# ceres-solver/ceres-solver

Measured on NVIDIA H100. Metric: lm_iterations_per_sec, higher is better.
Workload: dtype f64

## Files before the change

### ceres_solver_b200/csrc/b200ba.cu

```cuda
#include <algorithm>
#include <array>
#include <cmath>
#include <cstdarg>
#include <cstdio>
#include <cstdlib>
#include <cstring>
#include <limits>
#include <numeric>
#include <string>
#include <vector>

#ifdef B200_WITH_NCCL
#include <dlfcn.h>
#include <nccl.h>
#endif

#include "../../include/b200ba.h"
#include "kernels.cuh"
#include "kernels_v2.cuh"
#include "kernels_v2b.cuh"
#include "kernels_v4b.cuh"
#include "pmv_kernels.cuh"
#include "vector_kernels.cuh"
#include "cg_kernel.cuh"
// ... 189 lines not shown
  void* cusolver = nullptr;
  int num_huge = 0;
  int* d_huge_pts = nullptr;
  bool residuals_resident = false;
  double *d_ftf_inv = nullptr, *d_spse[3] = {nullptr, nullptr, nullptr};
  double *d_pq_parts = nullptr, *d_seed_pq = nullptr;
  int num_cam_items = 0;
  CamItem* d_cam_items = nullptr;
  int* d_cam_rows = nullptr;
  double* d_q3 = nullptr;
  bool xs = false;
  bool xs_ready = false;
  bool xs_diag_ready = false;
  int xs_grid = 0;
  XsView xsv{};
  int num_xs_long = 0, num_xs_short = 0;
  int* d_xs_order = nullptr;
  bool xs_pcg = false;
  XsPcgArgs xpa{};
  size_t xs_pcg_smem = 0;
  std::vector<int> h_cam_idx, h_pt_idx, h_pt_ptr;
  bool sp_ready = false;
  bool xs_arrays = false;
  SparseView spv{};
  long long sp_storage = 0;
  int sp_grid = 0;
  size_t sp_smem = 0;
  int* d_sp_cnt_init = nullptr;
  double* d_red = nullptr;
  bool xchg_ok = false;
  uint4* d_xchg = nullptr;
  XchgPeers xpeers{};
// ... 254 lines not shown
  OK(launch(h, K_SQNORM, [&] {
    sqnorm_kernel<<<h->grid_tile[K_SQNORM], kTile, tile_smem_bytes<3, 1>(), h->stream>>>(h->view, d_out);
  }));
  return allreduce_sum(h, d_out + 3 * static_cast<size_t>(h->P), 9 * static_cast<size_t>(h->C));
}

int scale_dev(b200_handle* h, const double* d_scale) {
  h->xs_ready = false;
  return launch(h, K_SCALE, [&] {
    scale_kernel<<<flat_grid(h, 12 * static_cast<size_t>(h->N), 256), 256, 0, h->stream>>>(h->view, d_scale);
  });
}

int xs_assemble_dev(b200_handle* h) {
  OK(launch(h, K_DIAG_BLOCKS, [&] {
    if (h->num_xs_long > 0)
      xs_assemble_kernel<true><<<std::min(h->num_xs_long, h->sm_count * 32), kXsAsmThreads, 0, h->stream>>>(
          h->xsv, h->view, h->d_xs_order, h->num_xs_long, h->d_ete_inv, h->d_upper45);
    if (h->num_xs_short > 0)
      xs_assemble_kernel<false><<<std::min((h->num_xs_short + kXsAsmThreads / 32 - 1) / (kXsAsmThreads / 32), h->sm_count * 32),
                                  kXsAsmThreads, 0, h->stream>>>(h->xsv, h->view, h->d_xs_order + h->num_xs_long, h->num_xs_short,
                                                                 h->d_ete_inv, h->d_upper45);
  }));
  h->xs_ready = true;
  h->xs_diag_ready = true;
  return B200_OK;
}

int schur_init_dev(b200_handle* h, const double* d_b, const double* d_D) {
  SchurState st{};
  st.b = d_b;
  st.D = d_D;
  st.ete_inv = h->d_ete_inv;
  st.rhs = h->d_rhs;
  st.ye = h->d_ye;
  CU(cudaMemsetAsync(h->d_rhs, 0, sizeof(double) * 9 * h->C, h->stream));
  h->q_from_init = false;
// ... 386 lines not shown
  summary->num_iterations = 1;
  summary->residual_norm = 0.0;
  if (h->h_fail[0] != 0 || h->h_fail[1] != 0) {
    summary->termination_type = B200_LS_FAILURE;
    return B200_OK;
  }
  summary->termination_type = B200_LS_SUCCESS;
  OK(back_substitute_dev(h, d_b, h->d_sol, d_x));
  CU(cudaMemcpyAsync(d_x + 3 * static_cast<size_t>(h->P), h->d_sol, sizeof(double) * n, cudaMemcpyDeviceToDevice, h->stream));
  return B200_OK;
}

constexpr double kFactorMaxBytes = 48.0 * (1ull << 30);
static_assert(kSpMaxCols == 9 * kSnMaxCams && kSpThreads == 32 * 8 && kSpTileRows == 64,
              "an update tile: two column blocks per warp, two rows per lane");
int sparse_analyse(b200_handle* h) {
  XsPattern xp;
  xs_pattern(h->C, h->N, h->h_cam_idx.data(), h->h_pt_idx.data(), h->h_pt_ptr.data(), &xp);
  SparsePlan sp;
  plan_sparse_schur(h->C, xp.blk_row, xp.blk_col, &sp);
  if (8.0 * static_cast<double>(sp.storage) > kFactorMaxBytes)
    return fail(B200_ERR_UNSUPPORTED, "sparse factor of %d cameras needs %.1f GB", h->C, 8.0 * static_cast<double>(sp.storage) / 1e9);
  if (!h->xs_arrays) {
    XsView& x = h->xsv;
    x.C = h->C;
    x.num_blocks = static_cast<int>(xp.blk_row.size());
    OK(upload(h, xp.blk_row, &x.blk_row));
    OK(upload(h, xp.blk_col, &x.blk_col));
    OK(upload(h, xp.pair_ptr, &x.pair_ptr));
    OK(upload(h, xp.pairs, &x.pairs));
    OK(dev_alloc(h, &x.S, 81 * static_cast<size_t>(x.num_blocks)));
    std::vector<int> order;
    h->num_xs_long = xs_assembly_order(xp, &order);
    h->num_xs_short = x.num_blocks - h->num_xs_long;
    OK(upload(h, order, &h->d_xs_order));
    h->xs_arrays = true;
  }
  SparseView& v = h->spv;
  v.C = h->C;
  v.ns = sp.ns;
  OK(upload(h, sp.pinv, &v.pinv));
  OK(upload(h, sp.sn_first, &v.sn_first));
  OK(upload(h, sp.row_ptr, &v.row_ptr));
  OK(upload(h, sp.rows, &v.rows));
  OK(upload(h, sp.val, &v.val));
  OK(upload(h, sp.upd_ptr, &v.upd_ptr));
  OK(upload(h, sp.upd, &v.upd));
  OK(upload(h, sp.ntf_ptr, &v.ntf_ptr));
  OK(upload(h, sp.ntf, &v.ntf));
  OK(upload(h, sp.blk_off, &v.blk_off));
// ... 322 lines not shown
  OK(raise_smem_limit(cam_blocks_v2_kernel<true>, (kCamBlkThreads / 32) * kCamBlkWarpBytes));
  OK(raise_smem_limit(cam_blocks_v2_kernel<false>, (kCamBlkThreads / 32) * kCamBlkWarpBytes));
  OK(raise_smem_limit(jtj_v2_kernel, lim));
  OK(raise_smem_limit(schur_mul_v3_kernel, lim));
  OK(raise_smem_limit(schur_init_v4_kernel<true>, lim));
  OK(raise_smem_limit(schur_init_v4_kernel<false>, lim));
  OK(raise_smem_limit(jtj_v4_kernel<true>, lim));
  OK(raise_smem_limit(jtj_v4_kernel<false>, lim));
  OK(raise_smem_limit(schur_mul_v4_kernel<true>, lim));
  OK(raise_smem_limit(schur_mul_v4_kernel<false>, lim));
  OK(raise_smem_limit(evaluate_v2_kernel<true>, lim));
  OK(raise_smem_limit(evaluate_v2_kernel<false>, lim));
  OK(raise_smem_limit(diag_blocks_v2_kernel<true>, lim));
  OK(raise_smem_limit(diag_blocks_v2_kernel<false>, lim));
  OK(raise_smem_limit(xs_pcg_kernel, lim));
  OK(raise_smem_limit(sparse_factor_kernel, lim));
  return B200_OK;
}

struct StepResult {
  b200_solver_summary ls{};
  double model_cost_change = 0.0;
  double step_sq = 0.0, x_sq = 0.0;
  bool finite = true;
};

struct DeviceSide {
  b200_handle* h;
  const b200_lm_options* opt;
  int np, vgrid;
// ... 742 lines not shown
      OK(upload(h, std::vector<int2>(pl.num_ctas, make_int2(0, 0)), &h->v2_mul.cta_big));
    }
    h->v2_smem = pl.v2_smem;
    h->mul_smem = pl.mul_smem;
    h->eval_v2_smem = pl.eval_smem;
    h->diag_v2_smem = pl.diag_smem;
    h->diag_v2_replicas = pl.diag_replicas;
  }
  if (h->xs) {
    const XsPattern& xp = pl.xp;
    XsView& x = h->xsv;
    x.C = C;
    x.num_blocks = static_cast<int>(xp.blk_row.size());
    OK(upload(h, xp.blk_row, &x.blk_row));
    OK(upload(h, xp.blk_col, &x.blk_col));
    OK(upload(h, xp.pair_ptr, &x.pair_ptr));
    OK(upload(h, xp.pairs, &x.pairs));
    OK(upload(h, xp.cols, &x.cols));
    OK(upload(h, xp.col_ptr, &x.col_ptr));
    OK(upload(h, pl.xs_steps, &x.steps));
    OK(upload(h, pl.xs_warp_step, &x.warp_step));
    OK(dev_alloc(h, &x.S, 81 * static_cast<size_t>(x.num_blocks)));
    OK(dev_alloc(h, &x.T, 9 * static_cast<size_t>(xp.off_blocks)));
    OK(upload(h, pl.xs_order, &h->d_xs_order));
    h->num_xs_long = pl.num_xs_long;
    h->num_xs_short = x.num_blocks - pl.num_xs_long;
    h->xs_grid = pl.xs_grid;
    h->xs_pcg = pl.xs_pcg;
    if (h->xs_pcg) {
      XsPcgArgs& a = h->xpa;
      a.v = x;
      OK(upload(h, pl.xs_pcg_cta, &a.cta));
      OK(upload(h, pl.xs_pcg_warp_step, &a.warp_step));
      OK(upload(h, pl.xs_pcg_fptr, &a.fptr));
      OK(upload(h, pl.xs_pcg_fcol, &a.fcol));
      OK(upload(h, pl.xs_pcg_cols, &a.v.cols));
      a.max_blocks = pl.xs_pcg_max_blocks;
      a.max_cams = pl.xs_pcg_max_cams;
      a.max_foreign = pl.xs_pcg_max_foreign;
      a.max_steps = pl.xs_pcg_max_cta_steps;
      a.stage_slots = pl.xs_pcg_stage_slots;
// ... 492 lines not shown
```

### ceres_solver_b200/csrc/common.cuh

```cuda
#pragma once
#include <cuda_runtime.h>
#include <stdint.h>

namespace b200 {

constexpr int kTile = 128;

struct TileDesc {
  int obs_begin = 0;
  int obs_count = 0;
  int pt_begin = 0;
  int pt_count = 0;
  int chunk = 0;
};

struct ProblemView {
  int C, P;
  int N;
  int num_tiles;
  const TileDesc* tiles;
  const int* cam_idx;
  const int* pt_ptr;
  const int* pt_of_row;
  const double* obs;
  double* values;
  __device__ __host__ double* E() const { return values; }
  __device__ __host__ double* F() const { return values + 6 * static_cast<size_t>(N); }
};

__device__ __forceinline__ uint32_t smem_u32(const void* p) {
  return static_cast<uint32_t>(__cvta_generic_to_shared(p));
}
__device__ __forceinline__ void mbar_init(uint64_t* bar, uint32_t count) {
  asm volatile("mbarrier.init.shared::cta.b64 [%0], %1;" ::"r"(smem_u32(bar)), "r"(count));
}
__device__ __forceinline__ void fence_mbar_init() {
  asm volatile("fence.mbarrier_init.release.cluster;" ::: "memory");
}
__device__ __forceinline__ void mbar_arrive_expect_tx(uint64_t* bar, uint32_t bytes) {
  asm volatile("mbarrier.arrive.expect_tx.shared::cta.b64 _, [%0], %1;" ::"r"(smem_u32(bar)), "r"(bytes)
               : "memory");
}
__device__ __forceinline__ bool mbar_try_wait(uint64_t* bar, uint32_t parity) {
  uint32_t ok;
  asm volatile(
      "{\n"
      ".reg .pred p;\n"
// ... 136 lines not shown
```

### ceres_solver_b200/csrc/explicit_schur.cuh

```cuda
#pragma once
#include "common.cuh"

namespace b200 {

constexpr int kXsThreads = 256;
constexpr int kXsWarps = kXsThreads / 32;
constexpr int kXsMinCtas = 2;
constexpr int kXsStep = 3;
constexpr int kXsAsmThreads = 256;
constexpr int kXsLongPairs = 96;
constexpr int kXsStepCountShift = 27;
constexpr int kXsStepFirst = 1 << 29;
constexpr int kXsStepLast = 1 << 30;

struct XsView {
  int C;
  int num_blocks;
  const int* blk_row;
  const int* blk_col;
  const int* pair_ptr;
  const int2* pairs;
  const int2* cols;
  const int* col_ptr;
  const int2* steps;
  const int* warp_step;
  double* S;
  double* T;
};

__device__ __forceinline__ void xs_pairs(const XsView& v, const ProblemView& p, const double* __restrict__ ete_inv, int q_begin,
                                         int q_end, int lane, double& acc0, double& acc1, double& acc2) {
  const double* __restrict__ E = p.E();
  const double* __restrict__ F = p.F();
  const bool owner = lane < 27;
  const int u = owner ? lane / 3 : 0, w0 = owner ? 3 * (lane - 3 * (lane / 3)) : 0;
  const int q = lane >> 2, ga = (lane >> 1) & 1, gc = lane & 1;
  for (int q0 = q_begin; q0 < q_end; q0 += 8) {
    const int nq = min(8, q_end - q0);
    int r = 0, s = 0;
    double g = 0.0;
    if (q < nq) {
      const int2 rs = __ldg(v.pairs + q0 + q);
      r = rs.x;
      s = rs.y;
      const double* er = E + 6 * static_cast<size_t>(r) + 3 * ga;
      const double* es = E + 6 * static_cast<size_t>(s) + 3 * gc;
      const double e0 = es[0], e1 = es[1], e2 = es[2], f0 = er[0], f1 = er[1], f2 = er[2];
      const double* pp = ete_inv + 6 * static_cast<size_t>(__ldg(p.pt_of_row + r));
      const double P00 = pp[0], P01 = pp[1], P02 = pp[2], P11 = pp[3], P12 = pp[4], P22 = pp[5];
      const double pe0 = P00 * e0 + P01 * e1 + P02 * e2;
      const double pe1 = P01 * e0 + P11 * e1 + P12 * e2;
      const double pe2 = P02 * e0 + P12 * e1 + P22 * e2;
      g = f0 * pe0 + f1 * pe1 + f2 * pe2;
      if (r == s && ga == gc) g -= 1.0;
    }
    for (int t0 = 0; t0 < nq; t0 += 4) {
      double fr[4][2], fs[4][6], gg[4][4];
#pragma unroll
      for (int t = 0; t < 4; ++t) {
        const int src = 4 * (t0 + t);
#pragma unroll
        for (int k = 0; k < 4; ++k) gg[t][k] = __shfl_sync(0xffffffffu, g, (src + k) & 31);
        const int rr = __shfl_sync(0xffffffffu, r, src & 31), ss = __shfl_sync(0xffffffffu, s, src & 31);
        const double* pr = F + 18 * static_cast<size_t>(rr) + u;
        const double* ps = F + 18 * static_cast<size_t>(ss) + w0;
        fr[t][0] = pr[0];
        fr[t][1] = pr[9];
#pragma unroll
        for (int m = 0; m < 3; ++m) {
          fs[t][m] = ps[m];
          fs[t][3 + m] = ps[9 + m];
        }
      }
#pragma unroll
      for (int t = 0; t < 4; ++t) {
        if (t0 + t >= nq) continue;
        const double a0 = gg[t][0] * fr[t][0] + gg[t][2] * fr[t][1], a1 = gg[t][1] * fr[t][0] + gg[t][3] * fr[t][1];
#pragma unroll
        acc0 -= a0 * fs[t][0] + a1 * fs[t][3];
        acc1 -= a0 * fs[t][1] + a1 * fs[t][4];
        acc2 -= a0 * fs[t][2] + a1 * fs[t][5];
      }
    }
  }
}

template <bool kLong>
__global__ void __launch_bounds__(kXsAsmThreads) xs_assemble_kernel(XsView v, ProblemView p, const int* __restrict__ blocks,
                                                                   int num, const double* __restrict__ ete_inv,
                                                                   double* __restrict__ upper45) {
  __shared__ double s_part[kLong ? kXsAsmThreads / 32 : 1][81];
  const int lane = threadIdx.x & 31, warp = threadIdx.x >> 5;
  const bool owner = lane < 27;
  const int u = owner ? lane / 3 : 0, w0 = owner ? 3 * (lane - 3 * (lane / 3)) : 0;
  const int item0 = kLong ? static_cast<int>(blockIdx.x) : static_cast<int>(blockIdx.x) * (kXsAsmThreads / 32) + warp;
  const int items = kLong ? static_cast<int>(gridDim.x) : static_cast<int>(gridDim.x) * (kXsAsmThreads / 32);
  for (int it = item0; it < num; it += items) {
    const int b = __ldg(blocks + it);
    const int p0 = __ldg(v.pair_ptr + b), p1 = __ldg(v.pair_ptr + b + 1);
    double acc[3] = {0.0, 0.0, 0.0};
    if (kLong) {
      constexpr int W = kXsAsmThreads / 32;
      const int n = p1 - p0;
      xs_pairs(v, p, ete_inv, p0 + static_cast<int>(static_cast<long long>(n) * warp / W),
               p0 + static_cast<int>(static_cast<long long>(n) * (warp + 1) / W), lane, acc[0], acc[1], acc[2]);
      __syncthreads();
      if (owner)
#pragma unroll
        for (int m = 0; m < 3; ++m) s_part[warp][9 * u + w0 + m] = acc[m];
      __syncthreads();
      if (warp != 0) continue;
      if (owner)
#pragma unroll
        for (int m = 0; m < 3; ++m) {
          double t = 0.0;
#pragma unroll
          for (int k = 0; k < W; ++k) t += s_part[k][9 * u + w0 + m];
          acc[m] = t;
        }
    } else {
      xs_pairs(v, p, ete_inv, p0, p1, lane, acc[0], acc[1], acc[2]);
    }
    if (owner) {
      double* sb = v.S + 81 * static_cast<size_t>(b) + 9 * u + w0;
      sb[0] = acc[0];
      sb[1] = acc[1];
      sb[2] = acc[2];
      const int i = __ldg(v.blk_row + b);
      if (upper45 != nullptr && __ldg(v.blk_col + b) == i) {
        double* o = upper45 + 45 * static_cast<size_t>(i) + u * 9 - u * (u - 1) / 2 - u;
        if (u <= w0) o[w0] = acc[0];
        if (u <= w0 + 1) o[w0 + 1] = acc[1];
        if (u <= w0 + 2) o[w0 + 2] = acc[2];
      }
    }
  }
}

struct XsStepData {
  int2 d;
  int2 c;
  double s[9];
};
template <bool kShared>
__device__ __forceinline__ int2 xs_step_desc(const XsView& v, int k, int k1) {
  return k < k1 ? (kShared ? v.steps[k] : __ldg(v.steps + k)) : make_int2(0, 0);
}
__device__ __forceinline__ bool xs_lane_in(int2 d, int e) { return e < ((d.y >> kXsStepCountShift) & 3); }
template <bool kShared>
__device__ __forceinline__ int2 xs_step_col(const XsView& v, int2 d, int e) {
// ... 147 lines not shown
```

### ceres_solver_b200/csrc/kernels_v4b.cuh

```cuda
#pragma once
#include "kernels_v2b.cuh"

namespace b200 {

__device__ __forceinline__ void invert_sym3_llt_rsqrt(const double m[6], double inv[6]) {
  const double i00 = rsqrt(m[0]);
  const double l10 = m[1] * i00, l20 = m[2] * i00;
  const double i11 = rsqrt(m[3] - l10 * l10);
  const double l21 = (m[4] - l20 * l10) * i11;
  const double i22 = rsqrt(m[5] - l20 * l20 - l21 * l21);
  const double i10 = -l10 * i00 * i11;
  const double i21 = -l21 * i11 * i22;
  const double i20 = -(l20 * i00 + l21 * i10) * i22;
  inv[0] = i00 * i00 + i10 * i10 + i20 * i20;
  inv[1] = i10 * i11 + i20 * i21;
  inv[2] = i20 * i22;
  inv[3] = i11 * i11 + i21 * i21;
  inv[4] = i21 * i22;
  inv[5] = i22 * i22;
}

struct InitV4Args {
  const double* b;
  const double* D;
// ... 280 lines not shown
    if (static_cast<int>(threadIdx.x) >= d.obs_count) continue;
    const size_t r = static_cast<size_t>(d.obs_begin) + threadIdx.x;
    const double2* ep = reinterpret_cast<const double2*>(p.E() + 6 * r);
    const double2 a0 = __ldg(ep), a1 = __ldg(ep + 1), a2 = __ldg(ep + 2);
    const double e00 = a0.x, e01 = a0.y, e02 = a1.x, e10 = a1.y, e11 = a2.x, e12 = a2.y;
    const double* pi = ete_inv + 6 * static_cast<size_t>(d.pt_begin);
    const double p0 = __ldg(pi), p1 = __ldg(pi + 1), p2 = __ldg(pi + 2), p3 = __ldg(pi + 3), p4 = __ldg(pi + 4), p5 = __ldg(pi + 5);
    const double a = p0 * e00 + p1 * e01 + p2 * e02, b = p1 * e00 + p3 * e01 + p4 * e02, c = p2 * e00 + p4 * e01 + p5 * e02;
    const double dd = p0 * e10 + p1 * e11 + p2 * e12, e = p1 * e10 + p3 * e11 + p4 * e12, f = p2 * e10 + p4 * e11 + p5 * e12;
    double2* q = reinterpret_cast<double2*>(q3 + kQStride * r);
    q[0] = make_double2(1.0 - (e00 * a + e01 * b + e02 * c), -(e10 * a + e11 * b + e12 * c));
    q[1] = make_double2(1.0 - (e10 * dd + e11 * e + e12 * f), 0.0);
  }
}

__device__ __forceinline__ void cp_async16(void* smem_dst, const void* gsrc) {
  asm volatile("cp.async.cg.shared.global [%0], [%1], 16;" ::"r"(smem_u32(smem_dst)), "l"(gsrc) : "memory");
}
__device__ __forceinline__ void cp_async_commit() { asm volatile("cp.async.commit_group;" ::: "memory"); }
template <int kPending>
__device__ __forceinline__ void cp_async_wait() { asm volatile("cp.async.wait_group %0;" ::"n"(kPending) : "memory"); }

constexpr int kCamBlkRowBytes = 144 + 32;
constexpr int kCamBlkDepth = 2;
constexpr int kCamBlkWarpBytes = kCamBlkDepth * 32 * kCamBlkRowBytes;
constexpr int kCamBlkThreads = 128;

__device__ __forceinline__ void cam_block_flush(double (&m)[46], double* dst) {
  const int lane = threadIdx.x & 31;
  int base = 0;
  double r1[23], r2[12], r3[6], r4[3], r5[2];
  {
    const bool up = (lane & 16) != 0;
#pragma unroll
    for (int k = 0; k < 23; ++k) {
      const double keep = up ? m[23 + k] : m[k], give = up ? m[k] : m[23 + k];
// ... 130 lines not shown
```

### ceres_solver_b200/csrc/plan.cuh

```cuda
#pragma once
#include <algorithm>
#include <cmath>
#include <cstdio>
#include <cstdlib>
#include <cstring>
#include <numeric>
#include <vector>

#include "explicit_schur.cuh"
#include "kernels_v4b.cuh"
#include "xs_pcg.cuh"

namespace b200 {

constexpr double kL2ResidentShare = 0.5;
constexpr double kXsByteRatio = 2.0;
constexpr double kXsMaxBytes = 128.0 * (1 << 20);

enum KernelId {
  K_EVAL_JAC = 0,
  K_EVAL_COST,
  K_SQNORM,
  K_SCALE,
  K_JMUL,
// ... 89 lines not shown
  int xs_ctas_per_sm;
  int xs_pcg_ctas_per_sm;
};

enum class MulFamily { Tile, V3, V4, V4Owned };
enum class DiagPass { CamMajor, WarpTile, Tile };

inline bool is_v4(MulFamily m) { return m == MulFamily::V4 || m == MulFamily::V4Owned; }

struct XsPattern {
  long long off_blocks = 0;
  std::vector<int> blk_row, blk_col, pair_ptr, row_ptr, col_ptr;
  std::vector<int2> pairs, cols;
};

struct KernelPlan {
  int order_choice = 0;
  long order_metrics[4] = {0, 0, 0, 0};
  std::vector<int> pt_perm;
  std::vector<int> row_perm;
  std::vector<int> cam_idx, pt_idx, pt_ptr;
  std::vector<double> obs;
  std::vector<TileDesc> tiles;
  std::vector<TileDesc> chunk_tiles;
  std::vector<int> huge_pts;
  std::vector<WarpTile> wtiles;
  std::vector<TileDesc> big_tiles;
  int num_plain_big = 0;
  std::vector<uint32_t> row_meta;
  std::vector<int> cam_rows;
// ... 1 lines not shown
  bool has_dups = false;
  int num_ctas = 0;
  std::vector<int2> cta_part, cta_cam, cta_big;
  std::vector<int> cta_cams;
  int max_cam_span = 1;
  MulFamily mul = MulFamily::Tile;
  DiagPass diag = DiagPass::Tile;
  bool big_folded = false;
  V2View v2{}, v2_mul{}, v2_eval{}, v2_diag{};
  size_t v2_smem = 0, mul_smem = 0, eval_smem = 0, diag_smem = 0;
  int diag_replicas = 0;
  std::vector<uint32_t> tile_meta;
  double l2_budget = 0.0, l2_stream_bytes = 0.0, l2_resident_bytes = 0.0;
  bool xs = false;
  XsPattern xp;
  std::vector<int> xs_order;
  std::vector<int2> xs_steps;
  std::vector<int> xs_warp_step;
  int num_xs_long = 0, xs_grid = 0, xs_resident = 0, xs_max_steps = 0;
  bool xs_pcg = false;
  std::vector<int2> xs_pcg_cta;
  std::vector<int> xs_pcg_warp_step;
  std::vector<int> xs_pcg_fptr;
  std::vector<int> xs_pcg_fcol;
  std::vector<int2> xs_pcg_cols;
  int xs_pcg_max_blocks = 0, xs_pcg_max_cams = 0, xs_pcg_max_steps = 0, xs_pcg_max_foreign = 0;
  int xs_pcg_max_cta_steps = 0;
  int xs_pcg_walk_max = 0;
  int xs_pcg_split_rows = 0;
  int xs_pcg_max_slots = 0;
  int xs_pcg_stage_slots = 0;
  size_t xs_pcg_smem = 0;
  const char* xs_pcg_why = "";
  double bytes_per_op[K_COUNT] = {};
// ... 45 lines not shown
    for (const int3& t : tup) xp->pairs[base + start[slot[t.x]]++] = make_int2(t.y, t.z);
  }
  const int nb = static_cast<int>(xp->blk_row.size());
  row_start[C] = nb;
  xp->pair_ptr.push_back(static_cast<int>(xp->pairs.size()));
  xp->col_ptr.assign(static_cast<size_t>(C) + 1, 0);
  for (int b = 0; b < nb; ++b)
    if (xp->blk_col[b] != xp->blk_row[b]) xp->col_ptr[xp->blk_col[b] + 1]++;
  for (int c = 0; c < C; ++c) xp->col_ptr[c + 1] += xp->col_ptr[c];
  std::vector<int> fill(xp->col_ptr.begin(), xp->col_ptr.end() - 1);
  xp->cols.resize(static_cast<size_t>(nb));
  for (int b = 0; b < nb; ++b)
    xp->cols[b] = make_int2(xp->blk_col[b], xp->blk_col[b] != xp->blk_row[b] ? fill[xp->blk_col[b]]++ : -1);
}

inline int xs_assembly_order(const XsPattern& xp, std::vector<int>* order) {
  const int nb = static_cast<int>(xp.blk_row.size());
  order->clear();
  order->reserve(static_cast<size_t>(nb));
  for (int b = 0; b < nb; ++b)
    if (xp.pair_ptr[b + 1] - xp.pair_ptr[b] > kXsLongPairs) order->push_back(b);
  const int num_long = static_cast<int>(order->size());
  for (int b = 0; b < nb; ++b)
    if (xp.pair_ptr[b + 1] - xp.pair_ptr[b] <= kXsLongPairs) order->push_back(b);
  return num_long;
}

const char* const kOrderNames[4] = {"caller's order kept", "by camera arc", "by mean camera", "by smallest camera"};
inline int choose_point_order(int C, int P, int N, const int32_t* cam_of_row, const int* caller_ptr, int chunks, std::vector<int>* perm,
                       long metrics[4]) {
  std::vector<int> ident(static_cast<size_t>(P));
  std::iota(ident.begin(), ident.end(), 0);
  auto metric = [&](const std::vector<int>& ord) -> long {
    std::vector<int> stamp(static_cast<size_t>(C), -1);
    long total = 0, rows = 0;
    int chunk = 0;
    const long target = N / chunks + 1;
    for (int k = 0; k < P; ++k) {
      const int q = ord[k];
      for (int r = caller_ptr[q]; r < caller_ptr[q + 1]; ++r) {
// ... 548 lines not shown
          if (!(dl & kXsStepLast) && ((df & kXsStepFirst) || (df & kXsStepRowMask) != (dl & kXsStepRowMask))) ++pl.xs_pcg_split_rows;
        }
      }
      for (int k = 0; k < G * kXpWarps; ++k)
        pl.xs_pcg_max_steps = std::max(pl.xs_pcg_max_steps, pl.xs_pcg_warp_step[k + 1] - pl.xs_pcg_warp_step[k]);
      const size_t base = xs_pcg_smem_bytes(pl.xs_pcg_max_blocks, pl.xs_pcg_max_cams, pl.xs_pcg_max_foreign, pl.xs_pcg_max_cta_steps, 0);
      const size_t room = lim.smem_optin > base + 1024 ? lim.smem_optin - base - 1024 : 0;
      pl.xs_pcg_stage_slots = static_cast<int>(std::min<size_t>(pl.xs_pcg_max_slots, room / (9 * sizeof(double))));
      pl.xs_pcg_smem = xs_pcg_smem_bytes(pl.xs_pcg_max_blocks, pl.xs_pcg_max_cams, pl.xs_pcg_max_foreign, pl.xs_pcg_max_cta_steps,
                                         pl.xs_pcg_stage_slots);
      if (pl.xs_pcg_smem + 1024 > lim.smem_optin) pl.xs_pcg_why = "largest CTA's shared memory exceeds the limit";
      else if (lim.xs_pcg_ctas_per_sm < 1) pl.xs_pcg_why = "no CTA of the kernel fits an SM";
      else if (knobs.xs_resident == 0) pl.xs_pcg_why = "B200_XS_RESIDENT=0";
      else pl.xs_pcg = true;
    }
    pl.num_xs_long = xs_assembly_order(xp, &pl.xs_order);
  }

  const double Nn = N, Pp = P, Cc = C;
  double* bpo = pl.bytes_per_op;
  bpo[K_JTJ] = 196 * Nn + 4 * Pp + 24.0 * (3 * Pp + 9 * Cc);
  bpo[K_SCHUR_MUL] = 196 * Nn + 52 * Pp + 216 * Cc;
  bpo[K_SCHUR_INIT] = 196 * Nn + 16 * Nn + 4 * Pp + 24 * Pp + 48 * Pp + 72 * Cc;
  bpo[K_DIAG_BLOCKS] = 196 * Nn + 52 * Pp + 360 * Cc;
  bpo[K_BACKSUB] = 196 * Nn + 16 * Nn + 52 * Pp + 24 * Pp + 72 * Cc;
  bpo[K_EVAL_JAC] = 192 * Nn + 16 * Nn + 16 * Nn + 4 * Nn + 4 * Pp + 2 * 8.0 * (3 * Pp + 9 * Cc);
  bpo[K_EVAL_COST] = 16 * Nn + 4 * Nn + 4 * Pp + 8.0 * (3 * Pp + 9 * Cc);
  bpo[K_SQNORM] = 196 * Nn + 4 * Pp + 8.0 * (3 * Pp + 9 * Cc);
  bpo[K_SCALE] = 2 * 192 * Nn + 8 * Nn + 8.0 * (3 * Pp + 9 * Cc);
  bpo[K_JMUL] = 196 * Nn + 32 * Nn + 4 * Pp + 8.0 * (3 * Pp + 9 * Cc);
  bpo[K_JTMUL] = 196 * Nn + 16 * Nn + 4 * Pp + 16.0 * (3 * Pp + 9 * Cc);
// ... 2 lines not shown
  bpo[K_PMV_LEFT_E] = 48 * Nn + 16 * Nn + 4 * Pp + 48 * Pp;
  bpo[K_PMV_LEFT_F] = 144 * Nn + 16 * Nn + 4 * Nn + 144 * Cc;
  bpo[K_MODEL_COST] = 196 * Nn + 16 * Nn + 4 * Pp + 8.0 * (3 * Pp + 9 * Cc);
  bpo[K_DOGLEG_GRAM] = 196 * Nn + 4 * Pp + 16.0 * (3 * Pp + 9 * Cc);
  bpo[K_DOGLEG_DIAG] = 48.0 * (3 * Pp + 9 * Cc);
  bpo[K_DOGLEG_GN] = 32.0 * (3 * Pp + 9 * Cc);
  bpo[K_DOGLEG_STEP] = 56.0 * (3 * Pp + 9 * Cc);
  if (pl.xs) {
    bpo[K_SCHUR_MUL] = xs_mul_bytes;
    bpo[K_DIAG_BLOCKS] = xs_asm_bytes;
    const double nb = static_cast<double>(pl.xp.blk_row.size()), off = static_cast<double>(pl.xp.off_blocks);
    if (pl.xs_pcg) bpo[K_SCHUR_PCG] = 656.0 * nb + 144.0 * off + 648.0 * Cc + 8 * 72.0 * Cc;
  }
}

inline void print_plan(const KernelPlan& pl, int C, int P, int N, int world, const DevLimits& lim, const DevKnobs& knobs) {
  if (getenv("B200_VERBOSE") == nullptr) return;
  if (!knobs.keep_order)
    fprintf(stderr, "[b200ba] point order: distinct cameras per 1/%d of the rows, summed: caller %ld, by camera arc %ld, by mean camera %ld, by smallest camera %ld -> %s\n",
            lim.sm_count, pl.order_metrics[0], pl.order_metrics[1], pl.order_metrics[2], pl.order_metrics[3], kOrderNames[pl.order_choice]);
  const V2View &v = pl.v2, &m = pl.v2_mul;
  if (is_v4(pl.mul)) {
    const uint32_t s = m.l2_stream;
    fprintf(stderr, "[b200ba] S*x L2 plan (L2 %d MiB, budget %.1f MiB): resident %.1f MiB, streamed %.1f MiB, stride %.2f tiles (%s)\n",
            lim.l2_bytes >> 20, pl.l2_budget / (1 << 20), pl.l2_resident_bytes / (1 << 20), (pl.l2_stream_bytes - pl.l2_resident_bytes) / (1 << 20),
            s < 65536 ? 65536.0 / (65536 - s) : 0.0, m.l2_last ? "evict_last" : "evict_normal");
  }
  const char* const mul_names[] = {"tile", "v3", "v4", "v4-owned"};
  const char* const diag_names[] = {"cam_major", "v2", "tile"};
  fprintf(stderr,
          "[b200ba] C=%d P=%d N=%d wtiles=%zu big(+slices)=%zu huge=%d span=%d direct=%d v2(w=%d,s=%d,r=%d) mul(%s w=%d,s=%d,r=%d,smem=%zu) folded=%d v2b=%d cam_major=%d diag=%s\n",
          C, P, N, pl.wtiles.size(), pl.big_tiles.size(), static_cast<int>(pl.huge_pts.size()), pl.max_cam_span, v.direct, v.warps, v.stages,
          v.replicas, mul_names[static_cast<int>(pl.mul)], m.warps, m.stages, m.replicas, pl.mul_smem, pl.big_folded ? 1 : 0,
          is_v4(pl.mul) ? 1 : 0, pl.diag == DiagPass::CamMajor ? 1 : 0, diag_names[static_cast<int>(pl.diag)]);
  if (world == 1) {
    fprintf(stderr, "[b200ba] S plan: %s, %lld pairs, %.1f MB\n", pl.xs ? "explicit" : "implicit", pl.xp.off_blocks,
            648.0 * static_cast<double>(pl.xp.blk_row.size()) / 1e6);
    if (pl.xs)
      fprintf(stderr, "[b200ba] S product: grid %d of %d resident CTAs (%d per SM), %d warps, at most %d steps per warp\n",
              pl.xs_grid, pl.xs_resident, lim.xs_ctas_per_sm, pl.xs_grid * kXsWarps, pl.xs_max_steps);
    if (pl.xs) {
      const double share = 648.0 * pl.xs_pcg_max_blocks / 1024.0, limit = static_cast<double>(lim.smem_optin) / 1024.0;
      const double cta = static_cast<double>(pl.xs_pcg_smem) / 1024.0;
      if (pl.xs_pcg) {
        fprintf(stderr, "[b200ba] S PCG: resident, %d CTAs, largest S share %.2f KiB of %.2f KiB (%.2f KiB with M^-1, vectors and staging), %d warps, at most %d steps per warp, at most %d foreign columns, at most %d column slots per CTA (%d staged)\n",
                lim.sm_count, share, limit, cta, lim.sm_count * kXpWarps, pl.xs_pcg_max_steps, pl.xs_pcg_max_foreign, pl.xs_pcg_max_slots,
                pl.xs_pcg_stage_slots);
        fprintf(stderr, "[b200ba] S PCG walk: at most %d steps per warp (one per row segment included), %d split rows\n",
                pl.xs_pcg_walk_max, pl.xs_pcg_split_rows);
      } else {
        fprintf(stderr, "[b200ba] S PCG: two-kernel (%s: largest S share %.2f KiB, %.2f KiB with M^-1, vectors and staging, of %.2f KiB)\n",
                pl.xs_pcg_why, share, cta, limit);
// ... 8 lines not shown
```

Baseline: 149.0.

## Assemble explicit Schur blocks per camera row with staged shared-memory F/E reuse

```diff
diff --git a/ceres_solver_b200/csrc/b200ba.cu b/ceres_solver_b200/csrc/b200ba.cu
--- a/ceres_solver_b200/csrc/b200ba.cu
+++ b/ceres_solver_b200/csrc/b200ba.cu
@@ -227,8 +227,7 @@
   bool xs_diag_ready = false;
   int xs_grid = 0;
   XsView xsv{};
-  int num_xs_long = 0, num_xs_short = 0;
-  int* d_xs_order = nullptr;
+  XaView xav{};
   bool xs_pcg = false;
   XsPcgArgs xpa{};
   size_t xs_pcg_smem = 0;
@@ -513,13 +512,7 @@
 
 int xs_assemble_dev(b200_handle* h) {
   OK(launch(h, K_DIAG_BLOCKS, [&] {
-    if (h->num_xs_long > 0)
-      xs_assemble_kernel<true><<<std::min(h->num_xs_long, h->sm_count * 32), kXsAsmThreads, 0, h->stream>>>(
-          h->xsv, h->view, h->d_xs_order, h->num_xs_long, h->d_ete_inv, h->d_upper45);
-    if (h->num_xs_short > 0)
-      xs_assemble_kernel<false><<<std::min((h->num_xs_short + kXsAsmThreads / 32 - 1) / (kXsAsmThreads / 32), h->sm_count * 32),
-                                  kXsAsmThreads, 0, h->stream>>>(h->xsv, h->view, h->d_xs_order + h->num_xs_long, h->num_xs_short,
-                                                                 h->d_ete_inv, h->d_upper45);
+    xs_assemble_kernel<<<h->C, kXaThreads, kXaSmem, h->stream>>>(h->xsv, h->xav, h->view, h->d_ete_inv, h->d_upper45);
   }));
   h->xs_ready = true;
   h->xs_diag_ready = true;
@@ -936,6 +929,20 @@
 constexpr double kFactorMaxBytes = 48.0 * (1ull << 30);
 static_assert(kSpMaxCols == 9 * kSnMaxCams && kSpThreads == 32 * 8 && kSpTileRows == 64,
               "an update tile: two column blocks per warp, two rows per lane");
+int upload_xs_assembly(b200_handle* h, const XsAsmPlan& xa) {
+  XaView& a = h->xav;
+  OK(upload(h, xa.rows, &a.rows));
+  OK(upload(h, xa.pairs, &a.pairs));
+  OK(upload(h, xa.stage_ptr, &a.stage_ptr));
+  OK(upload(h, xa.stages, &a.stages));
+  OK(upload(h, xa.warp_seg, &a.warp_seg));
+  OK(upload(h, xa.segs, &a.segs));
+  OK(upload(h, xa.long_ptr, &a.long_ptr));
+  OK(upload(h, xa.longs, &a.longs));
+  OK(dev_alloc(h, &a.part, 81 * kXaLongSegs * static_cast<size_t>(std::max(1, xa.num_long))));
+  return B200_OK;
+}
+
 int sparse_analyse(b200_handle* h) {
   XsPattern xp;
   xs_pattern(h->C, h->N, h->h_cam_idx.data(), h->h_pt_idx.data(), h->h_pt_ptr.data(), &xp);
@@ -949,13 +956,12 @@
     x.num_blocks = static_cast<int>(xp.blk_row.size());
     OK(upload(h, xp.blk_row, &x.blk_row));
     OK(upload(h, xp.blk_col, &x.blk_col));
-    OK(upload(h, xp.pair_ptr, &x.pair_ptr));
-    OK(upload(h, xp.pairs, &x.pairs));
     OK(dev_alloc(h, &x.S, 81 * static_cast<size_t>(x.num_blocks)));
-    std::vector<int> order;
-    h->num_xs_long = xs_assembly_order(xp, &order);
-    h->num_xs_short = x.num_blocks - h->num_xs_long;
-    OK(upload(h, order, &h->d_xs_order));
+    XsAsmPlan xa;
+    xs_assembly_plan(h->C, h->N, h->h_cam_idx.data(), h->h_pt_idx.data(), h->h_pt_ptr.data(), xp, &xa);
+    if (getenv("B200_VERBOSE") != nullptr) print_xs_assembly(xa);
+    OK(upload_xs_assembly(h, xa));
+    CU(cudaStreamSynchronize(h->stream));
     h->xs_arrays = true;
   }
   SparseView& v = h->spv;
@@ -1308,6 +1314,7 @@
   OK(raise_smem_limit(diag_blocks_v2_kernel<true>, lim));
   OK(raise_smem_limit(diag_blocks_v2_kernel<false>, lim));
   OK(raise_smem_limit(xs_pcg_kernel, lim));
+  OK(raise_smem_limit(xs_assemble_kernel, static_cast<int>(kXaSmem)));
   OK(raise_smem_limit(sparse_factor_kernel, lim));
   return B200_OK;
 }
@@ -2080,17 +2087,13 @@
     x.num_blocks = static_cast<int>(xp.blk_row.size());
     OK(upload(h, xp.blk_row, &x.blk_row));
     OK(upload(h, xp.blk_col, &x.blk_col));
-    OK(upload(h, xp.pair_ptr, &x.pair_ptr));
-    OK(upload(h, xp.pairs, &x.pairs));
     OK(upload(h, xp.cols, &x.cols));
     OK(upload(h, xp.col_ptr, &x.col_ptr));
     OK(upload(h, pl.xs_steps, &x.steps));
     OK(upload(h, pl.xs_warp_step, &x.warp_step));
     OK(dev_alloc(h, &x.S, 81 * static_cast<size_t>(x.num_blocks)));
     OK(dev_alloc(h, &x.T, 9 * static_cast<size_t>(xp.off_blocks)));
-    OK(upload(h, pl.xs_order, &h->d_xs_order));
-    h->num_xs_long = pl.num_xs_long;
-    h->num_xs_short = x.num_blocks - pl.num_xs_long;
+    OK(upload_xs_assembly(h, pl.xa));
     h->xs_grid = pl.xs_grid;
     h->xs_pcg = pl.xs_pcg;
     if (h->xs_pcg) {
diff --git a/ceres_solver_b200/csrc/common.cuh b/ceres_solver_b200/csrc/common.cuh
--- a/ceres_solver_b200/csrc/common.cuh
+++ b/ceres_solver_b200/csrc/common.cuh
@@ -31,6 +31,12 @@
 __device__ __forceinline__ uint32_t smem_u32(const void* p) {
   return static_cast<uint32_t>(__cvta_generic_to_shared(p));
 }
+__device__ __forceinline__ void cp_async16(void* smem_dst, const void* gsrc) {
+  asm volatile("cp.async.cg.shared.global [%0], [%1], 16;" ::"r"(smem_u32(smem_dst)), "l"(gsrc) : "memory");
+}
+__device__ __forceinline__ void cp_async_commit() { asm volatile("cp.async.commit_group;" ::: "memory"); }
+template <int kPending>
+__device__ __forceinline__ void cp_async_wait() { asm volatile("cp.async.wait_group %0;" ::"n"(kPending) : "memory"); }
 __device__ __forceinline__ void mbar_init(uint64_t* bar, uint32_t count) {
   asm volatile("mbarrier.init.shared::cta.b64 [%0], %1;" ::"r"(smem_u32(bar)), "r"(count));
 }
diff --git a/ceres_solver_b200/csrc/explicit_schur.cuh b/ceres_solver_b200/csrc/explicit_schur.cuh
--- a/ceres_solver_b200/csrc/explicit_schur.cuh
+++ b/ceres_solver_b200/csrc/explicit_schur.cuh
@@ -7,7 +7,6 @@
 constexpr int kXsWarps = kXsThreads / 32;
 constexpr int kXsMinCtas = 2;
 constexpr int kXsStep = 3;
-constexpr int kXsAsmThreads = 256;
 constexpr int kXsLongPairs = 96;
 constexpr int kXsStepCountShift = 27;
 constexpr int kXsStepFirst = 1 << 29;
@@ -18,8 +17,6 @@
   int num_blocks;
   const int* blk_row;
   const int* blk_col;
-  const int* pair_ptr;
-  const int2* pairs;
   const int2* cols;
   const int* col_ptr;
   const int2* steps;
@@ -28,112 +25,170 @@
   double* T;
 };
 
-__device__ __forceinline__ void xs_pairs(const XsView& v, const ProblemView& p, const double* __restrict__ ete_inv, int q_begin,
-                                         int q_end, int lane, double& acc0, double& acc1, double& acc2) {
+struct XaView {
+  const int* rows;
+  const int2* pairs;
+  const int* stage_ptr;
+  const int4* stages;
+  const int* warp_seg;
+  const int4* segs;
+  const int* long_ptr;
+  const int2* longs;
+  double* part;
+};
+
+constexpr int kXaThreads = 256;
+constexpr int kXaWarps = kXaThreads / 32;
+constexpr int kXaLongSegs = 8;
+constexpr int kXaRows = 96;
+constexpr int kXaPairs = 448;
+constexpr int kXaRowDoubles = 30;
+constexpr int kXaSegCost = 8;
+static_assert(kXaRows <= kXaThreads, "a thread per staged row");
+constexpr int kXaSelf = 1 << 30;
+constexpr int kXaFirst = 1, kXaLast = 2, kXaLong = 4, kXaDiag = 8;
+static_assert(kXaPairs <= 2 * kXaThreads, "at most two pairs per thread");
+constexpr size_t kXaSmem = sizeof(double) * ((18 + 6) * kXaPairs + kXaRowDoubles * kXaRows) + sizeof(int) * kXaPairs;
+
+__device__ __forceinline__ void xa_store(double* sb, double* upper45, int i, int u, int w0, const double* acc) {
+  sb[0] = acc[0];
+  sb[1] = acc[1];
+  sb[2] = acc[2];
+  if (upper45 != nullptr) {
+    double* o = upper45 + 45 * static_cast<size_t>(i) + u * 9 - u * (u - 1) / 2 - u;
+    if (u <= w0) o[w0] = acc[0];
+    if (u <= w0 + 1) o[w0 + 1] = acc[1];
+    if (u <= w0 + 2) o[w0 + 2] = acc[2];
+  }
+}
+
+struct XaSeg {
+  int4 d;
+  double* out;
+  double acc[3];
+};
+__device__ __forceinline__ void xa_seg_load(const XsView& v, const XaView& a, int sg, int g1, int u, int w0, bool owner, XaSeg& s) {
+  s.d = sg < g1 ? __ldg(a.segs + sg) : make_int4(0, 0, 0, kXaFirst);
+  s.out = ((s.d.w & kXaLong) ? a.part : v.S) + 81 * static_cast<size_t>(s.d.z) + 9 * u + w0;
+#pragma unroll
+  for (int m = 0; m < 3; ++m) s.acc[m] = !(s.d.w & kXaFirst) && owner ? s.out[m] : 0.0;
+}
+
+__global__ void __launch_bounds__(kXaThreads, 2) xs_assemble_kernel(XsView v, XaView a, ProblemView p,
+                                                                     const double* __restrict__ ete_inv, double* upper45) {
+  extern __shared__ __align__(16) double xa_smem[];
+  double* s_fs = xa_smem;
+  double* s_es = s_fs + 18 * kXaPairs;
+  double* s_row = s_es + 6 * kXaPairs;
+  int* s_rl = reinterpret_cast<int*>(s_row + kXaRowDoubles * kXaRows);
   const double* __restrict__ E = p.E();
   const double* __restrict__ F = p.F();
+  const int i = blockIdx.x, lane = threadIdx.x & 31, warp = threadIdx.x >> 5;
   const bool owner = lane < 27;
   const int u = owner ? lane / 3 : 0, w0 = owner ? 3 * (lane - 3 * (lane / 3)) : 0;
-  const int q = lane >> 2, ga = (lane >> 1) & 1, gc = lane & 1;
-  for (int q0 = q_begin; q0 < q_end; q0 += 8) {
-    const int nq = min(8, q_end - q0);
-    int r = 0, s = 0;
-    double g = 0.0;
-    if (q < nq) {
-      const int2 rs = __ldg(v.pairs + q0 + q);
-      r = rs.x;
-      s = rs.y;
-      const double* er = E + 6 * static_cast<size_t>(r) + 3 * ga;
-      const double* es = E + 6 * static_cast<size_t>(s) + 3 * gc;
-      const double e0 = es[0], e1 = es[1], e2 = es[2], f0 = er[0], f1 = er[1], f2 = er[2];
-      const double* pp = ete_inv + 6 * static_cast<size_t>(__ldg(p.pt_of_row + r));
+  const int st0 = __ldg(a.stage_ptr + i), st1 = __ldg(a.stage_ptr + i + 1);
+  for (int st = st0; st < st1; ++st) {
+    const int4 sd = __ldg(a.stages + st);
+    const int q0 = sd.x, np = sd.y - sd.x;
+    __syncthreads();
+    const int g0 = __ldg(a.warp_seg + kXaWarps * st + warp), g1 = __ldg(a.warp_seg + kXaWarps * st + warp + 1);
+    XaSeg nx;
+    xa_seg_load(v, a, g0, g1, u, w0, owner, nx);
+    if (threadIdx.x < sd.w) {
+      const int r = __ldg(a.rows + sd.z + threadIdx.x);
+      const double* pr = ete_inv + 6 * static_cast<size_t>(__ldg(p.pt_of_row + r));
+      double* dst = s_row + kXaRowDoubles * threadIdx.x;
+#pragma unroll
+      for (int m = 0; m < 9; ++m) cp_async16(dst + 2 * m, F + 18 * static_cast<size_t>(r) + 2 * m);
+#pragma unroll
+      for (int m = 0; m < 3; ++m) {
+        cp_async16(dst + 18 + 2 * m, E + 6 * static_cast<size_t>(r) + 2 * m);
+        cp_async16(dst + 24 + 2 * m, pr + 2 * m);
+      }
+    }
+    int2 prs[2];
+#pragma unroll
+    for (int j = 0; j < 2; ++j) {
+      const int t = threadIdx.x + j * kXaThreads;
+      prs[j] = t < np ? __ldg(a.pairs + q0 + t) : make_int2(0, 0);
+    }
+#pragma unroll
+    for (int j = 0; j < 2; ++j) {
+      const int t = threadIdx.x + j * kXaThreads;
+      if (t >= np) continue;
+      s_rl[t] = prs[j].x;
+      if (prs[j].x & kXaSelf) continue;
+#pragma unroll
+      for (int m = 0; m < 9; ++m) cp_async16(s_fs + 18 * t + 2 * m, F + 18 * static_cast<size_t>(prs[j].y) + 2 * m);
+#pragma unroll
+      for (int m = 0; m < 3; ++m) cp_async16(s_es + 6 * t + 2 * m, E + 6 * static_cast<size_t>(prs[j].y) + 2 * m);
+    }
+    cp_async_commit();
+    cp_async_wait<0>();
+    __syncthreads();
+#pragma unroll
+    for (int j = 0; j < 2; ++j) {
+      const int t = threadIdx.x + j * kXaThreads;
+      if (t >= np) continue;
+      const int rl = s_rl[t];
+      const double* er = s_row + kXaRowDoubles * (rl & (kXaSelf - 1)) + 18;
+      const double* pp = er + 6;
       const double P00 = pp[0], P01 = pp[1], P02 = pp[2], P11 = pp[3], P12 = pp[4], P22 = pp[5];
-      const double pe0 = P00 * e0 + P01 * e1 + P02 * e2;
-      const double pe1 = P01 * e0 + P11 * e1 + P12 * e2;
-      const double pe2 = P02 * e0 + P12 * e1 + P22 * e2;
-      g = f0 * pe0 + f1 * pe1 + f2 * pe2;
-      if (r == s && ga == gc) g -= 1.0;
-    }
-    for (int t0 = 0; t0 < nq; t0 += 4) {
-      double fr[4][2], fs[4][6], gg[4][4];
-#pragma unroll
-      for (int t = 0; t < 4; ++t) {
-        const int src = 4 * (t0 + t);
-#pragma unroll
-        for (int k = 0; k < 4; ++k) gg[t][k] = __shfl_sync(0xffffffffu, g, (src + k) & 31);
-        const int rr = __shfl_sync(0xffffffffu, r, src & 31), ss = __shfl_sync(0xffffffffu, s, src & 31);
-        const double* pr = F + 18 * static_cast<size_t>(rr) + u;
-        const double* ps = F + 18 * static_cast<size_t>(ss) + w0;
-        fr[t][0] = pr[0];
-        fr[t][1] = pr[9];
-#pragma unroll
-        for (int m = 0; m < 3; ++m) {
-          fs[t][m] = ps[m];
-          fs[t][3 + m] = ps[9 + m];
+      const double* es = (rl & kXaSelf) ? s_row + kXaRowDoubles * (rl & (kXaSelf - 1)) + 18 : s_es + 6 * t;
+      double g[4];
+#pragma unroll
+      for (int gc = 0; gc < 2; ++gc) {
+        const double e0 = es[3 * gc], e1 = es[3 * gc + 1], e2 = es[3 * gc + 2];
+        const double pe0 = P00 * e0 + P01 * e1 + P02 * e2;
+        const double pe1 = P01 * e0 + P11 * e1 + P12 * e2;
+        const double pe2 = P02 * e0 + P12 * e1 + P22 * e2;
+#pragma unroll
+        for (int ga = 0; ga < 2; ++ga) {
+          const double f0 = er[3 * ga], f1 = er[3 * ga + 1], f2 = er[3 * ga + 2];
+          double gv = f0 * pe0 + f1 * pe1 + f2 * pe2;
+          if ((rl & kXaSelf) && ga == gc) gv -= 1.0;
+          g[2 * ga + gc] = gv;
         }
       }
-#pragma unroll
-      for (int t = 0; t < 4; ++t) {
-        if (t0 + t >= nq) continue;
-        const double a0 = gg[t][0] * fr[t][0] + gg[t][2] * fr[t][1], a1 = gg[t][1] * fr[t][0] + gg[t][3] * fr[t][1];
-#pragma unroll
-        acc0 -= a0 * fs[t][0] + a1 * fs[t][3];
-        acc1 -= a0 * fs[t][1] + a1 * fs[t][4];
-        acc2 -= a0 * fs[t][2] + a1 * fs[t][5];
-      }
-    }
-  }
-}
-
-template <bool kLong>
-__global__ void __launch_bounds__(kXsAsmThreads) xs_assemble_kernel(XsView v, ProblemView p, const int* __restrict__ blocks,
-                                                                   int num, const double* __restrict__ ete_inv,
-                                                                   double* __restrict__ upper45) {
-  __shared__ double s_part[kLong ? kXsAsmThreads / 32 : 1][81];
-  const int lane = threadIdx.x & 31, warp = threadIdx.x >> 5;
-  const bool owner = lane < 27;
-  const int u = owner ? lane / 3 : 0, w0 = owner ? 3 * (lane - 3 * (lane / 3)) : 0;
-  const int item0 = kLong ? static_cast<int>(blockIdx.x) : static_cast<int>(blockIdx.x) * (kXsAsmThreads / 32) + warp;
-  const int items = kLong ? static_cast<int>(gridDim.x) : static_cast<int>(gridDim.x) * (kXsAsmThreads / 32);
-  for (int it = item0; it < num; it += items) {
-    const int b = __ldg(blocks + it);
-    const int p0 = __ldg(v.pair_ptr + b), p1 = __ldg(v.pair_ptr + b + 1);
-    double acc[3] = {0.0, 0.0, 0.0};
-    if (kLong) {
-      constexpr int W = kXsAsmThreads / 32;
-      const int n = p1 - p0;
-      xs_pairs(v, p, ete_inv, p0 + static_cast<int>(static_cast<long long>(n) * warp / W),
-               p0 + static_cast<int>(static_cast<long long>(n) * (warp + 1) / W), lane, acc[0], acc[1], acc[2]);
-      __syncthreads();
-      if (owner)
-#pragma unroll
-        for (int m = 0; m < 3; ++m) s_part[warp][9 * u + w0 + m] = acc[m];
-      __syncthreads();
-      if (warp != 0) continue;
-      if (owner)
-#pragma unroll
-        for (int m = 0; m < 3; ++m) {
-          double t = 0.0;
-#pragma unroll
-          for (int k = 0; k < W; ++k) t += s_part[k][9 * u + w0 + m];
-          acc[m] = t;
-        }
-    } else {
-      xs_pairs(v, p, ete_inv, p0, p1, lane, acc[0], acc[1], acc[2]);
-    }
-    if (owner) {
-      double* sb = v.S + 81 * static_cast<size_t>(b) + 9 * u + w0;
-      sb[0] = acc[0];
-      sb[1] = acc[1];
-      sb[2] = acc[2];
-      const int i = __ldg(v.blk_row + b);
-      if (upper45 != nullptr && __ldg(v.blk_col + b) == i) {
-        double* o = upper45 + 45 * static_cast<size_t>(i) + u * 9 - u * (u - 1) / 2 - u;
-        if (u <= w0) o[w0] = acc[0];
-        if (u <= w0 + 1) o[w0 + 1] = acc[1];
-        if (u <= w0 + 2) o[w0 + 2] = acc[2];
-      }
-    }
+      reinterpret_cast<double2*>(s_es + 6 * t)[0] = make_double2(g[0], g[1]);
+      reinterpret_cast<double2*>(s_es + 6 * t)[1] = make_double2(g[2], g[3]);
+    }
+    __syncthreads();
+    for (int sg = g0; sg < g1; ++sg) {
+      XaSeg cur = nx;
+      xa_seg_load(v, a, sg + 1, g1, u, w0, owner, nx);
+      const int ta = cur.d.x - q0, tb = cur.d.y - q0;
+#pragma unroll 4
+      for (int t = ta; t < tb; ++t) {
+        const double2 ga = reinterpret_cast<const double2*>(s_es + 6 * t)[0];
+        const double2 gb = reinterpret_cast<const double2*>(s_es + 6 * t)[1];
+        const int rl = s_rl[t];
+        const double* fr = s_row + kXaRowDoubles * (rl & (kXaSelf - 1)) + u;
+        const double* fs = ((rl & kXaSelf) ? fr - u : s_fs + 18 * t) + w0;
+        const double fr0 = fr[0], fr1 = fr[9];
+        const double a0 = ga.x * fr0 + gb.x * fr1, a1 = ga.y * fr0 + gb.y * fr1;
+        cur.acc[0] -= a0 * fs[0] + a1 * fs[9];
+        cur.acc[1] -= a0 * fs[1] + a1 * fs[10];
+        cur.acc[2] -= a0 * fs[2] + a1 * fs[11];
+      }
+      if (owner) xa_store(cur.out, (cur.d.w & kXaDiag) && (cur.d.w & kXaLast) ? upper45 : nullptr, i, u, w0, cur.acc);
+    }
+  }
+  const int l0 = __ldg(a.long_ptr + i), l1 = __ldg(a.long_ptr + i + 1);
+  if (l0 == l1) return;
+  __syncthreads();
+  for (int l = l0 + warp; l < l1; l += kXaWarps) {
+    const int2 lb = __ldg(a.longs + l);
+    if (!owner) continue;
+    double acc[3];
+#pragma unroll
+    for (int m = 0; m < 3; ++m) {
+      double t = 0.0;
+#pragma unroll
+      for (int k = 0; k < kXaLongSegs; ++k) t += a.part[81 * static_cast<size_t>(lb.y + k) + 9 * u + w0 + m];
+      acc[m] = t;
+    }
+    xa_store(v.S + 81 * static_cast<size_t>(lb.x) + 9 * u + w0, __ldg(v.blk_col + lb.x) == i ? upper45 : nullptr, i, u, w0, acc);
   }
 }
 
diff --git a/ceres_solver_b200/csrc/kernels_v4b.cuh b/ceres_solver_b200/csrc/kernels_v4b.cuh
--- a/ceres_solver_b200/csrc/kernels_v4b.cuh
+++ b/ceres_solver_b200/csrc/kernels_v4b.cuh
@@ -318,12 +318,6 @@
   }
 }
 
-__device__ __forceinline__ void cp_async16(void* smem_dst, const void* gsrc) {
-  asm volatile("cp.async.cg.shared.global [%0], [%1], 16;" ::"r"(smem_u32(smem_dst)), "l"(gsrc) : "memory");
-}
-__device__ __forceinline__ void cp_async_commit() { asm volatile("cp.async.commit_group;" ::: "memory"); }
-template <int kPending>
-__device__ __forceinline__ void cp_async_wait() { asm volatile("cp.async.wait_group %0;" ::"n"(kPending) : "memory"); }
 
 constexpr int kCamBlkRowBytes = 144 + 32;
 constexpr int kCamBlkDepth = 2;
diff --git a/ceres_solver_b200/csrc/plan.cuh b/ceres_solver_b200/csrc/plan.cuh
--- a/ceres_solver_b200/csrc/plan.cuh
+++ b/ceres_solver_b200/csrc/plan.cuh
@@ -127,6 +127,15 @@
   std::vector<int2> pairs, cols;
 };
 
+struct XsAsmPlan {
+  std::vector<int> rows, stage_ptr, warp_seg, long_ptr;
+  std::vector<int2> pairs, longs;
+  std::vector<int4> stages, segs;
+  int num_long = 0;
+  int max_rows = 0, max_pairs = 0;
+  long long max_load = 0;
+};
+
 struct KernelPlan {
   int order_choice = 0;
   long order_metrics[4] = {0, 0, 0, 0};
@@ -158,10 +167,10 @@
   double l2_budget = 0.0, l2_stream_bytes = 0.0, l2_resident_bytes = 0.0;
   bool xs = false;
   XsPattern xp;
-  std::vector<int> xs_order;
+  XsAsmPlan xa;
   std::vector<int2> xs_steps;
   std::vector<int> xs_warp_step;
-  int num_xs_long = 0, xs_grid = 0, xs_resident = 0, xs_max_steps = 0;
+  int xs_grid = 0, xs_resident = 0, xs_max_steps = 0;
   bool xs_pcg = false;
   std::vector<int2> xs_pcg_cta;
   std::vector<int> xs_pcg_warp_step;
@@ -237,16 +246,142 @@
     xp->cols[b] = make_int2(xp->blk_col[b], xp->blk_col[b] != xp->blk_row[b] ? fill[xp->blk_col[b]]++ : -1);
 }
 
-inline int xs_assembly_order(const XsPattern& xp, std::vector<int>* order) {
-  const int nb = static_cast<int>(xp.blk_row.size());
-  order->clear();
-  order->reserve(static_cast<size_t>(nb));
-  for (int b = 0; b < nb; ++b)
-    if (xp.pair_ptr[b + 1] - xp.pair_ptr[b] > kXsLongPairs) order->push_back(b);
-  const int num_long = static_cast<int>(order->size());
-  for (int b = 0; b < nb; ++b)
-    if (xp.pair_ptr[b + 1] - xp.pair_ptr[b] <= kXsLongPairs) order->push_back(b);
-  return num_long;
+
+inline void xs_assembly_plan(int C, int N, const int* cam_idx, const int* pt_idx, const int* pt_ptr, const XsPattern& xp,
+                             XsAsmPlan* out) {
+  XsAsmPlan& a = *out;
+  std::vector<int> cptr(static_cast<size_t>(C) + 1, 0);
+  for (int r = 0; r < N; ++r) cptr[cam_idx[r] + 1]++;
+  for (int c = 0; c < C; ++c) cptr[c + 1] += cptr[c];
+  a.rows.resize(static_cast<size_t>(N));
+  {
+    std::vector<int> fill(cptr.begin(), cptr.end() - 1);
+    for (int r = 0; r < N; ++r) a.rows[fill[cam_idx[r]]++] = r;
+  }
+  a.stage_ptr.assign(1, 0);
+  a.long_ptr.assign(1, 0);
+  a.warp_seg.clear();
+  std::vector<int> slot(static_cast<size_t>(C), 0), unit_base, unit_n, unit_seen, cnt, seg_of, bucket;
+  struct Walk { int unit, k, x, s; };
+  std::vector<Walk> walk, grouped;
+  std::vector<long long> cost;
+  for (int i = 0; i < C; ++i) {
+    const int b0 = xp.row_ptr[i], b1 = xp.row_ptr[i + 1];
+    unit_base.assign(static_cast<size_t>(b1 - b0) + 1, 0);
+    unit_n.clear();
+    for (int b = b0; b < b1; ++b) {
+      slot[xp.blk_col[b]] = b - b0;
+      const int n = xp.pair_ptr[b + 1] - xp.pair_ptr[b];
+      if (n > kXsLongPairs) {
+        a.longs.push_back(make_int2(b, kXaLongSegs * a.num_long++));
+        for (int k = 0; k < kXaLongSegs; ++k)
+          unit_n.push_back(static_cast<int>(static_cast<long long>(n) * (k + 1) / kXaLongSegs - static_cast<long long>(n) * k / kXaLongSegs));
+      } else {
+        unit_n.push_back(n);
+      }
+      unit_base[b - b0 + 1] = static_cast<int>(unit_n.size());
+    }
+    a.long_ptr.push_back(static_cast<int>(a.longs.size()));
+    const int nu = static_cast<int>(unit_n.size());
+    walk.clear();
+    cnt.assign(static_cast<size_t>(b1 - b0), 0);
+    seg_of.assign(static_cast<size_t>(b1 - b0), 0);
+    for (int k = cptr[i]; k < cptr[i + 1]; ++k) {
+      const int r = a.rows[k], p = pt_idx[r];
+      for (int s = pt_ptr[p]; s < pt_ptr[p + 1]; ++s) {
+        if (cam_idx[s] < i) continue;
+        const int bl = slot[cam_idx[s]], b = b0 + bl, n = xp.pair_ptr[b + 1] - xp.pair_ptr[b];
+        const int t = cnt[bl]++;
+        int u = unit_base[bl];
+        if (n > kXsLongPairs) {
+          while (static_cast<long long>(n) * (seg_of[bl] + 1) / kXaLongSegs <= t) ++seg_of[bl];
+          u += seg_of[bl];
+        }
+        walk.push_back(Walk{u, k - cptr[i], r == s ? kXaSelf : 0, s});
+      }
+    }
+    unit_seen.assign(static_cast<size_t>(nu), 0);
+    auto unit_out = [&](int u, int* flags) {
+      const int bl = static_cast<int>(std::upper_bound(unit_base.begin(), unit_base.end(), u) - unit_base.begin()) - 1;
+      const int b = b0 + bl;
+      if (unit_base[bl + 1] - unit_base[bl] > 1) {
+        *flags |= kXaLong;
+        const int l = static_cast<int>(std::lower_bound(a.longs.begin() + a.long_ptr[i], a.longs.end(), b,
+                                                        [](int2 e, int v) { return e.x < v; }) - a.longs.begin());
+        return a.longs[l].y + (u - unit_base[bl]);
+      }
+      if (b == b0) *flags |= kXaDiag;
+      return b;
+    };
+    auto add_stage = [&](size_t e0, size_t e1) {
+      const int k0 = e0 < e1 ? walk[e0].k : 0, nrows = e0 < e1 ? walk[e1 - 1].k - k0 + 1 : 0;
+      const int q0 = static_cast<int>(a.pairs.size());
+      a.stages.push_back(make_int4(q0, q0 + static_cast<int>(e1 - e0), cptr[i] + k0, nrows));
+      a.max_rows = std::max(a.max_rows, nrows);
+      a.max_pairs = std::max(a.max_pairs, static_cast<int>(e1 - e0));
+      bucket.assign(static_cast<size_t>(nu) + 1, 0);
+      for (size_t e = e0; e < e1; ++e) bucket[walk[e].unit + 1]++;
+      for (int u = 0; u < nu; ++u) bucket[u + 1] += bucket[u];
+      grouped.resize(e1 - e0);
+      {
+        std::vector<int> fill(bucket.begin(), bucket.end() - 1);
+        for (size_t e = e0; e < e1; ++e) grouped[fill[walk[e].unit]++] = walk[e];
+      }
+      const size_t s0 = a.segs.size();
+      cost.clear();
+      for (int u = 0; u < nu; ++u) {
+        const int n = bucket[u + 1] - bucket[u];
+        if (n == 0 && unit_n[u] > 0) continue;
+        int flags = (unit_seen[u] == 0 ? kXaFirst : 0) | (unit_seen[u] + n == unit_n[u] ? kXaLast : 0);
+        const int o = unit_out(u, &flags);
+        a.segs.push_back(make_int4(q0 + bucket[u], q0 + bucket[u + 1], o, flags));
+        cost.push_back(n + kXaSegCost);
+        unit_seen[u] += n;
+      }
+      for (const Walk& w : grouped) a.pairs.push_back(make_int2((w.k - k0) | w.x, w.s));
+      long long lo = 0, hi = 0;
+      for (long long c : cost) {
+        lo = std::max(lo, c);
+        hi += c;
+      }
+      auto fill = [&](long long K, int* ws) {
+        int g = 0;
+        long long load = 0;
+        if (ws != nullptr) ws[0] = static_cast<int>(s0);
+        for (size_t k = 0; k < cost.size(); ++k) {
+          if (load + cost[k] > K && load > 0) {
+            if (++g == kXaWarps) return g + 1;
+            if (ws != nullptr) ws[g] = static_cast<int>(s0 + k);
+            load = 0;
+          }
+          load += cost[k];
+        }
+        if (ws != nullptr)
+          while (g < kXaWarps - 1) ws[++g] = static_cast<int>(a.segs.size());
+        return g + 1;
+      };
+      while (lo < hi) {
+        const long long mid = lo + (hi - lo) / 2;
+        if (fill(mid, nullptr) <= kXaWarps) hi = mid;
+        else lo = mid + 1;
+      }
+      int ws[kXaWarps];
+      fill(lo, ws);
+      a.warp_seg.insert(a.warp_seg.end(), ws, ws + kXaWarps);
+      a.max_load = std::max(a.max_load, lo);
+    };
+    size_t e0 = 0;
+    for (size_t e = 0; e < walk.size(); ++e) {
+      const bool full = e - e0 == static_cast<size_t>(kXaPairs) || walk[e].k - walk[e0].k >= kXaRows;
+      if (full) {
+        add_stage(e0, e);
+        e0 = e;
+      }
+    }
+    if (e0 < walk.size() || walk.empty()) add_stage(e0, walk.size());
+    a.stage_ptr.push_back(static_cast<int>(a.stages.size()));
+  }
+  a.warp_seg.push_back(static_cast<int>(a.segs.size()));
 }
 
 const char* const kOrderNames[4] = {"caller's order kept", "by camera arc", "by mean camera", "by smallest camera"};
@@ -825,7 +960,7 @@
       else if (knobs.xs_resident == 0) pl.xs_pcg_why = "B200_XS_RESIDENT=0";
       else pl.xs_pcg = true;
     }
-    pl.num_xs_long = xs_assembly_order(xp, &pl.xs_order);
+    xs_assembly_plan(C, N, cam_idx, pt_idx, pt_ptr.data(), xp, &pl.xa);
   }
 
   const double Nn = N, Pp = P, Cc = C;
@@ -858,6 +993,11 @@
   }
 }
 
+inline void print_xs_assembly(const XsAsmPlan& a) {
+  fprintf(stderr, "[b200ba] S assembly: %zu stages, %zu segments, %d long blocks, largest warp load %lld (pairs + %d per segment), at most %d rows and %d pairs staged\n",
+          a.stages.size(), a.segs.size(), a.num_long, a.max_load, kXaSegCost, a.max_rows, a.max_pairs);
+}
+
 inline void print_plan(const KernelPlan& pl, int C, int P, int N, int world, const DevLimits& lim, const DevKnobs& knobs) {
   if (getenv("B200_VERBOSE") == nullptr) return;
   if (!knobs.keep_order)
@@ -880,6 +1020,7 @@
   if (world == 1) {
     fprintf(stderr, "[b200ba] S plan: %s, %lld pairs, %.1f MB\n", pl.xs ? "explicit" : "implicit", pl.xp.off_blocks,
             648.0 * static_cast<double>(pl.xp.blk_row.size()) / 1e6);
+    if (pl.xs) print_xs_assembly(pl.xa);
     if (pl.xs)
       fprintf(stderr, "[b200ba] S product: grid %d of %d resident CTAs (%d per SM), %d warps, at most %d steps per warp\n",
               pl.xs_grid, pl.xs_resident, lim.xs_ctas_per_sm, pl.xs_grid * kXsWarps, pl.xs_max_steps);
```

New measurement: 153.2 (median of 6 runs). 1.03x the previous value.
